# Sunefei/PathNet

Measured on AMD Instinct MI355X. Metric: paths aggregated/sec (PAGG fwd+bwd, one training step incl. on-GPU MERW sampling + Adam), higher is better.
Workload: dtype f32; 1 GPU; Cora-shaped synthetic (configs[1]): N=2708 F=1433 C=7 hid=128 path_num=40 path_len=4, 1299 masked nodes = 51960 paths/step, PathNet_homo, dropout 0.7, Adam; nodes=2708, parallelism=node-shard x1

## Files before the change

### pathnet_amd/csrc/pn_context.hip

```cpp
#include <hip/hip_runtime.h>

#include <cstdlib>
#include <cstring>
#include <map>
#include <new>
#include <vector>

#include "pn_internal.h"

struct pn_context {
    int device = 0;
    hipStream_t side = nullptr;
    hipEvent_t fork = nullptr, join = nullptr;
    int prof_mode = 0, prof_stage = -1;
    struct Rec {
        int stage;
        hipEvent_t a, b;
    };
    std::vector<Rec> recs;
    std::vector<hipEvent_t> free_events;
    std::map<const void *, int> lds_attr;
    pn::Knobs knobs;
};

namespace {

__global__ void warm_kernel() {}

__global__ void step_state_advance_kernel(pn_step_state *s) {
    if (threadIdx.x != 0 || blockIdx.x != 0) return;
    s->epoch += 1;
    s->adam_step += 1;
    uint64_t z = (s->seed += 0x9E3779B97F4A7C15ull);
    z = (z ^ (z >> 30)) * 0xBF58476D1CE4E5B9ull;
    z = (z ^ (z >> 27)) * 0x94D049BB133111EBull;
    s->seed = z ^ (z >> 31);
// ... 22 lines not shown
    (void)hipEventCreateWithFlags(&e, ctx->knobs.event_dev ? hipEventDisableSystemFence : hipEventDefault);
    return e;
}

}

namespace {

struct KnobName {
    const char *name;
    int pn::Knobs::*field;
};
const KnobName kKnobs[] = {{"PN_NODE_GEMM3", &pn::Knobs::node_gemm3}, {"PN_EVAL_ZW", &pn::Knobs::eval_zw},
                           {"PN_POOL_STEP", &pn::Knobs::pool_step}, {"PN_EVENT_DEVICE_SCOPE", &pn::Knobs::event_dev},
                           {"PN_NODE_RGRAD", &pn::Knobs::node_rgrad}, {"PN_SAMPLER_STAGE", &pn::Knobs::sampler_stage},
                           {"PN_SEQ4", &pn::Knobs::seq4}, {"PN_FC0_SPARSE", &pn::Knobs::fc0_sparse}};

}

namespace pn {

const Knobs &knobs_of(const pn_context *ctx) {
    static const Knobs defaults;
    return ctx ? ctx->knobs : defaults;
}

bool profiling_every_stage(const pn_context *ctx) { return ctx && ctx->prof_mode == 1; }

int context_check_device(const pn_context *ctx) {
    if (!ctx) return PN_OK;
    int dev = -1;
    PN_CHECK_HIP(hipGetDevice(&dev));
    if (dev != ctx->device)
        PN_FAIL(PN_ERR_ARG, "pn_context belongs to device %d, the current device is %d", ctx->device, dev);
    return PN_OK;
}

int ensure_dynamic_lds(pn_context *ctx, const void *kernel, int bytes) {
    if (ctx) {
        auto it = ctx->lds_attr.find(kernel);
        if (it != ctx->lds_attr.end() && it->second >= bytes) return PN_OK;
    }
    PN_CHECK_HIP(hipFuncSetAttribute(kernel, hipFuncAttributeMaxDynamicSharedMemorySize, bytes));
    if (ctx) ctx->lds_attr[kernel] = bytes;
    return PN_OK;
}

void *context_side_stream(pn_context *ctx) { return ctx ? (void *)ctx->side : nullptr; }
void *context_fork(pn_context *ctx, void *stream) {
    if (!ctx || !ctx->side) return nullptr;
    if (hipEventRecord(ctx->fork, (hipStream_t)stream) != hipSuccess) return nullptr;
    if (hipStreamWaitEvent(ctx->side, ctx->fork, 0) != hipSuccess) return nullptr;
    return ctx->side;
}
int context_record_join(pn_context *ctx) {
    PN_CHECK_HIP(hipEventRecord(ctx->join, ctx->side));
    return PN_OK;
}
int context_join(pn_context *ctx, void *stream) {
// ... 178 lines not shown
```

### pathnet_amd/csrc/pn_internal.h

```cpp
#pragma once
#include <cstdarg>
#include <cstdint>
#include <cstdio>

#include "../../include/pathnet_hip.h"

namespace pn {

void set_error(const char *fmt, ...) __attribute__((format(printf, 1, 2)));

#define PN_FAIL(code, ...)          \
    do {                            \
        ::pn::set_error(__VA_ARGS__); \
        return (code);              \
    } while (0)

#define PN_CHECK_HIP(expr)                                                                      \
    do {                                                                                        \
        hipError_t e_ = (expr);                                                                 \
        if (e_ != hipSuccess) PN_FAIL(PN_ERR_HIP, "%s failed: %s", #expr, hipGetErrorString(e_)); \
    } while (0)

struct GlibcPoly {
    uint32_t c[31];
// ... 4 lines not shown
GlibcPoly glibc_poly_one();
GlibcPoly glibc_poly_mul(const GlibcPoly &a, const GlibcPoly &b);
GlibcPoly glibc_poly_xpow(uint64_t d);
GlibcState glibc_apply(const GlibcPoly &p, const GlibcState &st);
GlibcState glibc_seed_state(uint32_t seed);

struct Knobs {
    int node_gemm3 = 7;
    int eval_zw = 1;
    int event_dev = 1;
    int pool_step = 1;
    int node_rgrad = 1;
    int sampler_stage = -1;
    int seq4 = 4;
    int fc0_sparse = 1;
};
const Knobs &knobs_of(const pn_context *ctx);

enum Stage {
    ST_SAMPLER_FILL = 0, ST_SAMPLER_WALK, ST_GATHER, ST_FC0, ST_BANK, ST_PLAN_PACK, ST_SEQ_FWD, ST_POOL_FWD,
    ST_FC2_GRAD, ST_POOL_BWD, ST_SEQ_BWD, ST_WGRAD, ST_BIAS_GRAD, ST_BANK_BWD, ST_FC0_BWD, ST_ZERO_FILL, ST_COUNT
};
bool profiling_every_stage(const pn_context *ctx);
int context_check_device(const pn_context *ctx);
void *context_fork(pn_context *ctx, void *stream);
void *context_side_stream(pn_context *ctx);
int context_record_join(pn_context *ctx);
int context_join(pn_context *ctx, void *stream);
int context_wait_side(pn_context *ctx, void *stream);
int ensure_dynamic_lds(pn_context *ctx, const void *kernel, int bytes);
struct StageTimer {
    StageTimer(pn_context *ctx, int stage, void *stream);
    ~StageTimer();
    pn_context *ctx;
    int slot;
    void *stream;
};

struct ZeroList {
    float *ptr[12];
    unsigned long long count[12];
    int n;
};
struct ZeroFill {
    pn_context *ctx;
// ... 24 lines not shown
```

### pathnet_amd/csrc/pn_pagg.hip

```cpp
#include <hip/hip_runtime.h>

#include <algorithm>
#include <cstdlib>
#include <cstring>
#include "pn_det.h"
#include "pn_gemm.h"
#include "pn_internal.h"
#include "pn_loss.h"
#include "pn_plan.h"
#include "pn_pool.h"
#include "pn_seq.h"
#include "pn_sparse.h"

using namespace pn;

namespace {

enum { CELL_LSTM = 1, CELL_RNN = 2, CELL_GRU = 3, CELL_MEAN = 4, CELL_SUM = 5 };
struct Dims {
    int variant, N, F, H, C, S, W, L, G, SV;
    int cell, Gw;
    int gru;
    bool generic;
    int S_total, group_begin;
// ... 80 lines not shown

inline size_t align256(size_t x) { return (x + 255) / 256 * 256; }

WsLayout ws_layout(const Dims &d) {
    WsLayout w{};
    const size_t N = d.N, H = d.H, L = d.L, G = d.G, SV = d.SV, Sb = d.Sb, Pb = (size_t)d.Sb * d.W;
    size_t at = 0;
    auto take = [&](size_t bytes) {
        size_t o = at;
        at = align256(at + bytes);
        return o;
    };
    w.Xh = take(N * H * 4);
    w.Z = take((size_t)d.ZR * H * 4);
    w.range = take(sizeof(SeqRange));
    w.wmax = take(64 * 4);
    w.Wp = take(G * H * 3 * H * 4);
    w.biasc = take(G * H * 4);
    w.WpT = take(G * H * 3 * H * 4);
    {
        const size_t rows = Pb * L, tiles = std::max<size_t>(1, ((G * H + WG_BM - 1) / WG_BM) * ((2 * H + WG_BN - 1) / WG_BN));
        const double wg_flops = 2.0 * (double)rows * (double)(G * H) * (double)(2 * H);
        size_t cus = wg_flops <= 1.2e11 ? WGRAD_CUS_SHARED : 256;
        size_t nz = (cus + tiles - 1) / tiles;
        const size_t max_nz = (rows + 4 * WG_KT - 1) / (4 * WG_KT);
        if (nz > max_nz) nz = max_nz;
        if (nz < 1) nz = 1;
        w.wgrad_split = (int)nz;
        w.wgrad_tiles = (int)tiles;
        w.wpart = take(nz * (G * H * 2 * H + G * H) * 4);
    }
// ... 282 lines not shown
    sp.L = d.L;
    sp.Pmask = d.P_total;
    sp.p_drop = a->p_seq;
    sp.seed = a->seed;
    sp.dyn = a->step_state;
    sp.mask = a->mask_seq;
    StageTimer tm(c.ctx, ST_SEQ_FWD, c.stream);
    if (!save && use_zw(c)) {
        sp.range = c.at<SeqRange>(c.w.range);
        sp.ZW = c.at<const float>(c.w.saved);
        return launch_seq_fwdzw(c.ctx, c.stream, d.H, d.Gw, sp);
    }
    if (d.math == PN_SEQ_MATH_F16X2) {
        sp.range = c.at<SeqRange>(c.w.range);
        sp.xmul = seq_xmul(a);
        return launch_seq_fwdh(c.ctx, c.stream, d.H, d.Gw, sp);
    }
    return launch_seq_fwd3(c.ctx, c.stream, d.H, d.Gw, sp);
}

PoolParams pool_fwd_params(const Call &c, int b, float *out) {
    const Dims &d = c.d;
    const pn_pagg_args *a = c.a;
    const int homo = d.variant == PN_VARIANT_HOMO;
    PoolParams pp{};
    pp.variant = d.variant;
    pp.S = c.groups(b);
    pp.W = d.W;
    pp.H = d.H;
    pp.C = d.C;
// ... 789 lines not shown
```

### pathnet_amd/csrc/pn_seq.h

```cpp
#pragma once
#include <cstdint>

#include "pn_internal.h"

namespace pn {

struct SeqRange {
    uint32_t x;
    int32_t x_esum;
    uint32_t x_cnt;
    uint32_t w_ih, w_hh;
    uint32_t dg;
};

struct SeqFwdParams {
    const float *Z;
    const int32_t *rowidx;
    const int32_t *slotof;
    const float *Wp;
    const float *biasc;
    float *hn;
    float *saved;
    float *xh;
    uint8_t *keep;
    int P, L;
    int64_t Pmask;
    float p_drop;
    uint64_t seed;
    const pn_step_state *dyn;
    const float *mask;
    const SeqRange *range;
    float xmul;
    const float *ZW;
};

struct SeqBwdParams {
    const float *saved;
    const uint8_t *keep;
    const float *dhn;
    const int32_t *rowidx, *slotof;
    const float *WpT;
    float *dG;
    float *dZ;
    int P, L;
    int merge0;
    int64_t Pmask;
    float p_drop;
    uint64_t seed;
    const float *mask;
// ... 101 lines not shown
```

### pathnet_amd/csrc/pn_seq_core.h

```cpp
#pragma once
#include <hip/hip_runtime.h>

#include <type_traits>

#include "pn_internal.h"
#include "pn_kernels.h"
#include "pn_seq.h"

namespace pn {

struct LstmFwd {
    float ig, fg, gg, og, c, h;
};
__device__ __forceinline__ LstmFwd lstm_fwd(float pi, float pf, float pg, float po, float cprev) {
    LstmFwd o;
    o.ig = sigmoidf_(pi);
    o.fg = sigmoidf_(pf);
    o.gg = tanhf_(pg);
    o.og = sigmoidf_(po);
    o.c = o.fg * cprev + o.ig * o.gg;
    o.h = o.og * tanhf_(o.c);
    return o;
}
struct GruFwd {
// ... 89 lines not shown
}
__device__ __forceinline__ float keep_dx(float dx, uint32_t keep_byte, int col, float keep_scale) {
    return (keep_byte >> (col & 3)) & 1 ? dx * keep_scale : 0.0f;
}

template <int H_, int GC_, int PLANES_>
struct SeqTile {
    static constexpr int H = H_, GC = GC_, PLANES = PLANES_;
    static constexpr int G = GC == 3 ? 4 : GC;
    static constexpr bool GRU = GC == 3;
    static constexpr int MT = 32, NW = H / 32, NT = NW * 64, GH = G * H;
    static constexpr int SV = G == 4 ? 5 : 1;
    static constexpr int FWD_PB = 4 * H + 16, FWD_PLANE = MT * FWD_PB;
    static __device__ __forceinline__ int *fwd_rowidx(unsigned char *lds) { return reinterpret_cast<int *>(lds + PLANES * FWD_PLANE); }
    static __device__ __forceinline__ int *fwd_slotof(unsigned char *lds, int L) { return fwd_rowidx(lds) + MT * L; }
    static constexpr int fwd_lds_bytes(int L) { return PLANES * FWD_PLANE + (MT * L + MT) * 4; }
    static constexpr int ZW_PB = 2 * H + 16, ZW_PLANE = MT * ZW_PB;
    static __device__ __forceinline__ int *zw_rowidx(unsigned char *lds) { return reinterpret_cast<int *>(lds + PLANES * ZW_PLANE); }
    static constexpr int zw_lds_bytes(int L) { return PLANES * ZW_PLANE + MT * L * 4; }
    static constexpr int NPASS = PLANES == 3 && G == 4 ? 2 : 1, KP = GH / NPASS;
    static constexpr int BWD_PB = 2 * KP + 16, BWD_PLANE = MT * BWD_PB, SMAX = PLANES == 2 ? 8 : 0;
    static __device__ __forceinline__ int *bwd_rowidx(unsigned char *lds) { return reinterpret_cast<int *>(lds + PLANES * BWD_PLANE); }
    static __device__ __forceinline__ int *bwd_slotof(unsigned char *lds, int L) { return bwd_rowidx(lds) + MT * L; }
    static __device__ __forceinline__ float *bwd_smax(unsigned char *lds, int L) { return reinterpret_cast<float *>(bwd_slotof(lds, L) + MT); }
    static __device__ __forceinline__ uint8_t *bwd_keep(unsigned char *lds, int L) { return reinterpret_cast<uint8_t *>(bwd_smax(lds, L) + SMAX); }
    static constexpr int bwd_lds_bytes(int L) { return PLANES * BWD_PLANE + (MT * L + MT) * 4 + SMAX * 4 + 2 * MT * (H / 4); }
};

template <class F>
int dispatch_seq(int H, int gc, F &&f) {
    auto by_h = [&](auto gcc) {
// ... 8 lines not shown
            case 256: return f(std::integral_constant<int, 256>{}, gcc);
        }
        PN_FAIL(PN_ERR_ARG, "hidden size %d not supported", H);
    };
    return gc == 3 ? by_h(std::integral_constant<int, 3>{}) : gc == 4 ? by_h(std::integral_constant<int, 4>{})
                                                                     : by_h(std::integral_constant<int, 1>{});
}

template <class... KArgs, class... Args>
int launch_with_lds(pn_context *ctx, void *stream, void (*kern)(KArgs...), dim3 grid, dim3 block, int lds_bytes, const Args &...args) {
    if (int rc = ensure_dynamic_lds(ctx, reinterpret_cast<const void *>(kern), lds_bytes)) return rc;
    hipLaunchKernelGGL(kern, grid, block, (size_t)lds_bytes, (hipStream_t)stream, args...);
    PN_CHECK_HIP(hipGetLastError());
    return PN_OK;
}
template <class T, class Params>
int launch_seq_tiles(pn_context *ctx, void *stream, void (*kern)(Params), int lds_bytes, const Params &sp) {
    return launch_with_lds(ctx, stream, kern, dim3((sp.P + T::MT - 1) / T::MT), dim3(T::NT), lds_bytes, sp);
}

}
```

### pathnet_amd/csrc/pn_seqh.hip

```cpp
#include <hip/hip_runtime.h>

#include <cstdlib>
#include <type_traits>

#include "pn_kernels.h"
#include "pn_seq.h"
#include "pn_seq_core.h"

using namespace pn;

#ifndef PN_FWDH_WAVES
#define PN_FWDH_WAVES 3
#endif
#ifndef PN_BWDH_WAVES
#define PN_BWDH_WAVES 2
#endif
#ifndef PN_TRACE_H
#define PN_TRACE_H 0
#endif
#if PN_TRACE_H
__device__ long long *g_trace_h = nullptr;
#define HSTAMP(slot)                                                                                      \
    do {                                                                                                  \
        if (g_trace_h && threadIdx.x == 0 && (slot) < 64)                                                 \
            g_trace_h[(size_t)blockIdx.x * 64 + (slot)] = (long long)__builtin_readcyclecounter();        \
    } while (0)
#define HSTAMP_RT(slot)                                                                                   \
    do {                                                                                                  \
        if (g_trace_h && threadIdx.x == 0)                                                                \
            g_trace_h[(size_t)blockIdx.x * 64 + (slot)] = (long long)__builtin_amdgcn_s_memrealtime();    \
    } while (0)
#else
#define HSTAMP(slot) do { } while (0)
#define HSTAMP_RT(slot) do { } while (0)
#endif

namespace {

typedef int i32x4 __attribute__((ext_vector_type(4)));

__device__ __forceinline__ uint32_t fbits_abs(float v) { return __float_as_uint(v) & 0x7fffffffu; }

constexpr int RANGE_PARTS = 32;
__global__ __launch_bounds__(256) void range_part_kernel(const float *__restrict__ w_ih, const float *__restrict__ w_hh, int64_t n4,
                                                         int clear_x, SeqRange *__restrict__ range, uint32_t *__restrict__ part) {
    __shared__ float red[2][4];
    const int64_t per = (n4 + RANGE_PARTS - 1) / RANGE_PARTS, lo = (int64_t)blockIdx.x * per, hi = min(n4, lo + per);
    float m0 = 0.0f, m1 = 0.0f;
    for (int64_t i = lo + threadIdx.x; i < hi; i += 256) {
        const float4 a = reinterpret_cast<const float4 *>(w_ih)[i], b = reinterpret_cast<const float4 *>(w_hh)[i];
        m0 = fmaxf(m0, fmaxf(fmaxf(fabsf(a.x), fabsf(a.y)), fmaxf(fabsf(a.z), fabsf(a.w))));
        m1 = fmaxf(m1, fmaxf(fmaxf(fabsf(b.x), fabsf(b.y)), fmaxf(fabsf(b.z), fabsf(b.w))));
    }
    m0 = wave_max(m0);
    m1 = wave_max(m1);
    if ((threadIdx.x & 63) == 0) red[0][threadIdx.x >> 6] = m0, red[1][threadIdx.x >> 6] = m1;
    __syncthreads();
    if (threadIdx.x == 0) {
        part[blockIdx.x] = __float_as_uint(fmaxf(fmaxf(red[0][0], red[0][1]), fmaxf(red[0][2], red[0][3])));
        part[RANGE_PARTS + blockIdx.x] = __float_as_uint(fmaxf(fmaxf(red[1][0], red[1][1]), fmaxf(red[1][2], red[1][3])));
        if (blockIdx.x == 0) {
            range->dg = 0u;
            if (clear_x) {
                range->x = 0u;
                range->x_esum = 0;
                range->x_cnt = 0u;
            }
        }
    }
}
__device__ __forceinline__ void range_from_parts(const uint32_t *__restrict__ part, float &m_ih, float &m_hh) {
    const int lane = threadIdx.x & 63;
    const float v = __uint_as_float(part[lane]);
    static_assert(2 * RANGE_PARTS == 64, "one partial per lane");
    float a = lane < RANGE_PARTS ? v : 0.0f, b = lane < RANGE_PARTS ? 0.0f : v;
    m_ih = wave_max(a);
    m_hh = wave_max(b);
// ... 78 lines not shown
constexpr int fwdh_waves() { return H == 32 ? 1 : H > 128 ? 2 : PN_FWDH_WAVES; }

template <int H, int GC>
__global__ __launch_bounds__(H / 32 * 64, (fwdh_waves<H>())) void seq_fwdh_kernel(SeqFwdParams p) {
    using T = SeqTile<H, GC, 2>;
    constexpr int G = T::G, MT = T::MT, NT = T::NT;
    constexpr bool GRU = T::GRU;
    constexpr bool PACKED = GC == 4;
    constexpr int SV = PACKED ? 4 : T::SV;
    constexpr int KS = H / 8, KX = KS / 2;
    constexpr int PB = T::FWD_PB, PLANE = T::FWD_PLANE;
    constexpr bool PREFETCH_X = fwdh_waves<H>() < 3, PING_PONG = PREFETCH_X;
    extern __shared__ __attribute__((aligned(16))) unsigned char ldsb[];
    int *s_rowidx = T::fwd_rowidx(ldsb);
    int *s_slotof = T::fwd_slotof(ldsb, p.L);
    const int tid = threadIdx.x, wave = tid >> 6, lane = tid & 63, li = lane & 31;
    const int q0 = __builtin_amdgcn_readfirstlane((int)blockIdx.x * MT);
    const int rows_here = __builtin_amdgcn_readfirstlane(min(MT, p.P - q0));
    const int col = 32 * wave + li;
    const int wave_u = __builtin_amdgcn_readfirstlane(wave);

    for (int i = tid; i < MT * p.L; i += NT) s_rowidx[i] = i / p.L < rows_here ? p.rowidx[(int64_t)q0 * p.L + i] : 0;
    for (int i = tid; i < MT; i += NT) s_slotof[i] = i < rows_here ? p.slotof[q0 + i] : 0;

    const FwdScales sc = fwd_scales(p.range, p.xmul);
    f32x16 cst;
#pragma unroll
    for (int r = 0; r < 16; r++) cst[r] = 0.0f;
    const float keep_scale = __int_as_float(__builtin_amdgcn_readfirstlane(__float_as_int(1.0f / (1.0f - p.p_drop))));
    const bool builtin_drop = !p.mask && p.p_drop > 0.0f;
    const uint64_t seed = p.dyn ? p.dyn->seed : p.seed;
    const size_t tile_row = (size_t)q0 * (size_t)p.L;
    uint8_t *keep_t = p.keep ? p.keep + tile_row * (H / 4) : nullptr;
    float4 *xh4_t = p.xh ? reinterpret_cast<float4 *>(p.xh) + tile_row * (2 * H / 4) : nullptr;
    float *xh_t = p.xh ? p.xh + tile_row * (2 * H) : nullptr;
    float *saved_t = p.saved ? p.saved + tile_row * (SV * H) : nullptr;
    float *hn_t = p.hn + (size_t)q0 * H;
    __syncthreads();

    constexpr int NLD = 4;
    f32x4 xr[NLD];
    uint32_t keepbits = 0;
    int tid_g = tid;
    auto gather_issue = [&](int t) {
#pragma unroll
        for (int i = 0; i < NLD; i++) {
            const int idx = tid_g + NT * i;
            const int row = idx / (H / 4), c4 = idx - row * (H / 4);
            async_load_b128(xr[i], p.Z + ((size_t)(uint32_t)s_rowidx[row * p.L + t] * (H / 4) + c4) * 4);
        }
        uint32_t bits = 0;
        if (builtin_drop) {
#pragma unroll
            for (int i = 0; i < NLD; i++) {
                const int idx = tid_g + NT * i;
                const int row = idx / (H / 4), c4 = idx - row * (H / 4);
                const float4 m = dropout4(seed, ((uint64_t)t * p.Pmask + s_slotof[row]) * (H / 4) + c4, 1u, p.p_drop);
                bits |= keep_nibble(m) << (4 * i);
            }
        }
        asm volatile("" : "+v"(bits));
        keepbits = bits;
    };
    auto gather_commit = [&](int t) {
        wait_vm<0>(xr[0], xr[1], xr[2], xr[3]);
#pragma unroll
        for (int i = 0; i < NLD; i++) {
            const int idx = tid_g + NT * i;
            const int row = idx / (H / 4), c4 = idx - row * (H / 4);
            const bool live = row < rows_here;
            float4 v = make_float4(xr[i][0], xr[i][1], xr[i][2], xr[i][3]);
            if (!live) v = make_float4(0.f, 0.f, 0.f, 0.f);
            if (p.mask) {
                if (live) {
                    const float4 m = reinterpret_cast<const float4 *>(
                        p.mask)[((int64_t)t * p.Pmask + s_slotof[row]) * (H / 4) + c4];
                    v.x *= m.x; v.y *= m.y; v.z *= m.z; v.w *= m.w;
                }
            } else if (builtin_drop) {
                const uint32_t b = keepbits >> (4 * i);
                v.x = b & 1u ? v.x * keep_scale : 0.0f;
                v.y = b & 2u ? v.y * keep_scale : 0.0f;
                v.z = b & 4u ? v.z * keep_scale : 0.0f;
                v.w = b & 8u ? v.w * keep_scale : 0.0f;
                if (keep_t && live) keep_t[((uint32_t)row * (uint32_t)p.L + t) * (uint32_t)(H / 4) + c4] = (uint8_t)(b & 15u);
            }
            uint32_t a0, a1, b0, b1;
            split2h(v.x * sc.s_x, v.y * sc.s_x, a0, a1);
            split2h(v.z * sc.s_x, v.w * sc.s_x, b0, b1);
            unsigned char *d = ldsb + row * PB + 8 * c4;
            *reinterpret_cast<uint2 *>(d) = make_uint2(a0, b0);
            *reinterpret_cast<uint2 *>(d + PLANE) = make_uint2(a1, b1);
            if (xh4_t && live) {
                float4 *xo = &at_bytes(xh4_t, (((uint32_t)row * (uint32_t)p.L + t) * (uint32_t)(2 * H / 4) + c4) * 16u);
                xo[0] = v;
                if (t == 0) xo[H / 4] = make_float4(0.f, 0.f, 0.f, 0.f);
            }
        }
    };
    gather_issue(0);
    gather_commit(0);
    __syncthreads();

    for (int t = 0; t < p.L; t++) {
        if (t == 0) HSTAMP_RT(62);
        HSTAMP(4 * t + 0);
        tid_g = wave_u * 64 + fresh_lane();
        if (PREFETCH_X && t + 1 < p.L) gather_issue(t + 1);

        f32x16 acc[G];
#pragma unroll
        for (int g = 0; g < G; g++) {
            const float bias = p.biasc[g * H + col] * sc.S;
#pragma unroll
            for (int r = 0; r < 16; r++) acc[g][r] = bias;
        }

        {
            const int nsteps = t == 0 ? KX : KS;
            const unsigned char *wb = reinterpret_cast<const unsigned char *>(p.Wp) + (size_t)wave_u * (KS * 2 * G * 1024);
            const int lane_k = fresh_lane();
            const uint32_t voff = lane_k * 16;
            const unsigned char *arow = ldsb + (lane_k & 31) * PB + 16 * (lane_k >> 5);
            u32x4 Bha[G], Bhb[G], Bl[G];
            auto load = [&](u32x4 (&B)[G], int s, int pl) {
                async_load_frags<G>(B, wb + (size_t)(s * 2 + pl) * (G * 1024), voff);
            };
            u32x4 a[2];
            auto areads = [&](int s, int pl) { a[pl] = *reinterpret_cast<const u32x4 *>(arow + 32 * s + pl * PLANE); };
            auto prod = [&](int pa, u32x4 (&B)[G]) {
#pragma unroll
                for (int g = 0; g < G; g++) acc[g] = mfma_f16(a[pa], B[g], acc[g]);
            };
            auto kstep = [&](int s, u32x4 (&Bh)[G], u32x4 (&Bhnext)[G]) {
                const int sn = min(s + 1, nsteps - 1);
                if (PING_PONG) load(Bhnext, sn, 0);
                wait_frag<(PING_PONG ? 2 : 1) * G, G>(Bh);
                prod(1, Bh);
                areads(sn, 1);
                prod(0, Bh);
                if (!PING_PONG) load(Bh, sn, 0);
                wait_frag<G, G>(Bl);
                prod(0, Bl);
                areads(sn, 0);
                load(Bl, sn, 1);
            };
            areads(0, 0);
            areads(0, 1);
            load(Bha, 0, 0);
            load(Bl, 0, 1);
#pragma unroll 1
            for (int s = 0; s < nsteps; s += 2) {
                if (PING_PONG) {
                    kstep(s, Bha, Bhb);
                    kstep(s + 1, Bhb, Bha);
                } else {
                    kstep(s, Bha, Bha);
                    kstep(s + 1, Bha, Bha);
                }
            }
            wait_frag<0, G>(Bha);
            wait_frag<0, G>(Bl);
        }
        HSTAMP(4 * t + 1);
        __syncthreads();
        HSTAMP(4 * t + 2);

        const int lane_o = fresh_lane();
        float hv[16];
#pragma unroll
        for (int r = 0; r < 16; r++) {
            const int row = acc_row(r, lane_o);
            const bool live = row < rows_here;
            float h;
            if (GRU) {
                const float hp = cst[r];
                const GruFwd c = gru_fwd(acc[0][r] * sc.inv_S, acc[G > 1 ? 1 : 0][r] * sc.inv_S, acc[G > 2 ? 2 : 0][r] * sc.inv_S,
                                         acc[G > 3 ? 3 : 0][r] * sc.inv_S, hp);
                h = c.h;
                cst[r] = h;
                if (saved_t && live) {
                    float *sv = &at_bytes(saved_t, (((uint32_t)row * (uint32_t)p.L + t) * (uint32_t)(SV * H) + col) * 4u);
                    sv[0] = c.rg; sv[H] = c.zg; sv[2 * H] = c.ng; sv[3 * H] = c.nh; sv[4 * H] = hp;
                }
            } else if (G == 4) {
                const float cprev = cst[r];
                const LstmFwd c = lstm_fwd(acc[0][r] * sc.inv_S, acc[G > 1 ? 1 : 0][r] * sc.inv_S, acc[G > 2 ? 2 : 0][r] * sc.inv_S,
                                           acc[G > 3 ? 3 : 0][r] * sc.inv_S, cprev);
                cst[r] = c.c;
                h = c.h;
                if (saved_t && live) {
                    const uint32_t base = ((uint32_t)row * (uint32_t)p.L + t) * (uint32_t)(SV * H);
                    const uint3 pk = pack_gates(c.ig, c.fg, c.gg, c.og);
                    *reinterpret_cast<uint4 *>(&at_bytes(saved_t, (base + 4u * col) * 4u)) =
                        make_uint4(pk.x, pk.y, pk.z, __float_as_uint(cprev));
                }
            } else {
                h = rnn_fwd(acc[0][r] * sc.inv_S);
                if (saved_t && live) at_bytes(saved_t, (((uint32_t)row * (uint32_t)p.L + t) * (uint32_t)H + col) * 4u) = h;
            }
            hv[r] = h;
            if (live) {
                if (t == p.L - 1)
                    at_bytes(hn_t, ((uint32_t)row * (uint32_t)H + col) * 4u) = h;
                else if (xh_t)
                    at_bytes(xh_t, (((uint32_t)row * (uint32_t)p.L + t + 1) * (uint32_t)(2 * H) + H + col) * 4u) = h;
            }
        }
        if (t + 1 < p.L) {
#pragma unroll
            for (int r = 0; r < 16; r += 2) {
                uint32_t h0, h1;
                split2h(hv[r] * sc.s_h, hv[r + 1] * sc.s_h, h0, h1);
                unsigned char *d = ldsb + acc_row(r, lane_o) * PB + 2 * (H + col);
                *reinterpret_cast<uint16_t *>(d) = (uint16_t)h0;
                *reinterpret_cast<uint16_t *>(d + PB) = (uint16_t)(h0 >> 16);
                *reinterpret_cast<uint16_t *>(d + PLANE) = (uint16_t)h1;
                *reinterpret_cast<uint16_t *>(d + PLANE + PB) = (uint16_t)(h1 >> 16);
            }
        }
        if (t + 1 < p.L) {
            tid_g = wave_u * 64 + fresh_lane();
            if (!PREFETCH_X) gather_issue(t + 1);
            gather_commit(t + 1);
            __syncthreads();
        }
        HSTAMP(4 * t + 3);
    }
    HSTAMP_RT(63);
}

template <int H, int GC>
__global__ __launch_bounds__(H / 32 * 64, (fwdh_waves<H>())) void seq_fwdzw_kernel(SeqFwdParams p) {
    using T = SeqTile<H, GC, 2>;
    constexpr int G = T::G, MT = T::MT, NT = T::NT, GH = T::GH;
    constexpr bool GRU = T::GRU;
    constexpr int KS = H / 8, KX = KS / 2, KH = KS - KX;
    constexpr int PB = T::ZW_PB, PLANE = T::ZW_PLANE;
    constexpr bool PING_PONG = fwdh_waves<H>() < 3;
    extern __shared__ __attribute__((aligned(16))) unsigned char ldsb[];
    int *s_rowidx = T::zw_rowidx(ldsb);
    const int tid = threadIdx.x, wave = tid >> 6, lane = tid & 63, li = lane & 31;
    const int q0 = blockIdx.x * MT;
    const int col = 32 * wave + li;
// ... 146 lines not shown
    constexpr bool GRU = T::GRU;
    constexpr bool PACKED = GC == 4;
    constexpr int SV = PACKED ? 4 : T::SV;
    constexpr int PB = T::BWD_PB, PLANE = T::BWD_PLANE;
    constexpr int NU = GH / 32;
    extern __shared__ __attribute__((aligned(16))) unsigned char ldsb[];
    int *s_rowidx = T::bwd_rowidx(ldsb);
    int *s_slotof = T::bwd_slotof(ldsb, p.L);
    float *s_max = T::bwd_smax(ldsb, p.L);
    uint8_t *s_keep = T::bwd_keep(ldsb, p.L);
    const int tid = threadIdx.x, wave = tid >> 6, lane = tid & 63, li = lane & 31;
    const int q0 = __builtin_amdgcn_readfirstlane((int)(gridDim.x - 1 - blockIdx.x) * MT);
    const int rows_here = __builtin_amdgcn_readfirstlane(min(MT, p.P - q0));
    const int col = 32 * wave + li;
    const int wave_u = __builtin_amdgcn_readfirstlane(wave);

    const int nidx = MT * p.L;
    auto rowidx_of = [&](int i) {
        const int rc = min(i & (MT - 1), rows_here - 1);
        return p.rowidx[((int64_t)q0 + rc) * p.L + i / MT];
    };
    const int ri0 = rowidx_of(min(tid, nidx - 1));
    const int sl0 = p.slotof[q0 + min(tid, rows_here - 1)];

    const float keep_scale = __int_as_float(__builtin_amdgcn_readfirstlane(__float_as_int(1.0f / (1.0f - p.p_drop))));
    const int e_ih = scale_exp(__uint_as_float(p.range->w_ih)), e_hh = scale_exp(__uint_as_float(p.range->w_hh));
    const size_t tile_row = (size_t)q0 * (size_t)p.L;
    const float *saved_t = p.saved + tile_row * (SV * H);
    float *dG_t = p.dG + tile_row * GH;
    const uint8_t *keep_t = p.keep ? p.keep + tile_row * (H / 4) : nullptr;
// ... 445 lines not shown
    hipLaunchKernelGGL(range_part_kernel, dim3(RANGE_PARTS), dim3(256), 0, s, w_ih, w_hh, (int64_t)Gw * H * H / 4, clear_x, range,
                       reinterpret_cast<uint32_t *>(part));
    PN_CHECK_HIP(hipGetLastError());
    const int nb = (G * H * H / 4 + 255) / 256;
    hipLaunchKernelGGL(pack_fb_kernel, dim3((unsigned)(WpT ? 2 * nb : nb)), dim3(256), 0, s, w_ih, w_hh, b_ih, b_hh, H, G, gru,
                       reinterpret_cast<const uint32_t *>(part), range, nb, reinterpret_cast<u32x4 *>(Wp), biasc,
                       reinterpret_cast<u32x4 *>(WpT));
    PN_CHECK_HIP(hipGetLastError());
    return PN_OK;
}

int launch_seq_fwdh(pn_context *ctx, void *stream, int H, int gc, const SeqFwdParams &sp) {
    if (!sp.range) PN_FAIL(PN_ERR_ARG, "seq_fwdh: operand ranges missing");
    return dispatch_seq(H, gc, [&](auto h, auto g) {
        using T = SeqTile<h.value, g.value, 2>;
        return launch_seq_tiles<T>(ctx, stream, seq_fwdh_kernel<h.value, g.value>, T::fwd_lds_bytes(sp.L), sp);
    });
}

int launch_seq_fwdzw(pn_context *ctx, void *stream, int H, int gc, const SeqFwdParams &sp) {
    if (!sp.range || !sp.ZW) PN_FAIL(PN_ERR_ARG, "seq_fwdzw: operand ranges / ZW missing");
    return dispatch_seq(H, gc, [&](auto h, auto g) {
        using T = SeqTile<h.value, g.value, 2>;
        return launch_seq_tiles<T>(ctx, stream, seq_fwdzw_kernel<h.value, g.value>, T::zw_lds_bytes(sp.L), sp);
    });
}

int launch_seq_bwdh(pn_context *ctx, void *stream, int H, int gc, const SeqBwdParams &sp) {
    if (!sp.range) PN_FAIL(PN_ERR_ARG, "seq_bwdh: operand ranges missing");
    return dispatch_seq(H, gc, [&](auto h, auto g) {
        using T = SeqTile<h.value, g.value, 2>;
// ... 12 lines not shown
```

Baseline: 61.72 million paths/s.

## Make forward sequence kernel persistent with atomic tile queue

Converts the f16x2 forward sequence kernel into a persistent kernel. The grid is sized to the resident block slots from an occupancy query, and blocks pull further tiles from a global atomic ticket counter, which resets itself when the last block leaves. The aim is to cut the tail and launch imbalance that come from launching one block per tile. In exchange it adds atomics, per-tile re-reads of kernel arguments, extra LDS for the ticket, and more register pressure from the restructured loop.

```diff
diff --git a/pathnet_amd/csrc/pn_context.hip b/pathnet_amd/csrc/pn_context.hip
--- a/pathnet_amd/csrc/pn_context.hip
+++ b/pathnet_amd/csrc/pn_context.hip
@@ -4,6 +4,7 @@
 #include <cstring>
 #include <map>
 #include <new>
+#include <utility>
 #include <vector>
 
 #include "pn_internal.h"
@@ -20,6 +21,8 @@
     std::vector<Rec> recs;
     std::vector<hipEvent_t> free_events;
     std::map<const void *, int> lds_attr;
+    std::map<std::pair<const void *, int>, int> slots;
+    int cus = 0;
     pn::Knobs knobs;
 };
 
@@ -72,7 +75,8 @@
 const KnobName kKnobs[] = {{"PN_NODE_GEMM3", &pn::Knobs::node_gemm3}, {"PN_EVAL_ZW", &pn::Knobs::eval_zw},
                            {"PN_POOL_STEP", &pn::Knobs::pool_step}, {"PN_EVENT_DEVICE_SCOPE", &pn::Knobs::event_dev},
                            {"PN_NODE_RGRAD", &pn::Knobs::node_rgrad}, {"PN_SAMPLER_STAGE", &pn::Knobs::sampler_stage},
-                           {"PN_SEQ4", &pn::Knobs::seq4}, {"PN_FC0_SPARSE", &pn::Knobs::fc0_sparse}};
+                           {"PN_SEQ4", &pn::Knobs::seq4}, {"PN_FC0_SPARSE", &pn::Knobs::fc0_sparse},
+                           {"PN_SEQ_GRID", &pn::Knobs::seq_grid}};
 
 }
 
@@ -101,6 +105,29 @@
     }
     PN_CHECK_HIP(hipFuncSetAttribute(kernel, hipFuncAttributeMaxDynamicSharedMemorySize, bytes));
     if (ctx) ctx->lds_attr[kernel] = bytes;
+    return PN_OK;
+}
+
+int resident_slots(pn_context *ctx, const void *kernel, int threads, int lds_bytes, int *slots) {
+    const std::pair<const void *, int> key(kernel, lds_bytes);
+    if (ctx) {
+        auto it = ctx->slots.find(key);
+        if (it != ctx->slots.end()) {
+            *slots = it->second;
+            return PN_OK;
+        }
+    }
+    int cus = ctx ? ctx->cus : 0;
+    if (cus <= 0) {
+        int dev = 0;
+        PN_CHECK_HIP(hipGetDevice(&dev));
+        PN_CHECK_HIP(hipDeviceGetAttribute(&cus, hipDeviceAttributeMultiprocessorCount, dev));
+        if (ctx) ctx->cus = cus;
+    }
+    int per_cu = 0;
+    PN_CHECK_HIP(hipOccupancyMaxActiveBlocksPerMultiprocessor(&per_cu, kernel, threads, (size_t)lds_bytes));
+    *slots = (per_cu > 0 ? per_cu : 1) * (cus > 0 ? cus : 1);
+    if (ctx) ctx->slots[key] = *slots;
     return PN_OK;
 }
 
diff --git a/pathnet_amd/csrc/pn_internal.h b/pathnet_amd/csrc/pn_internal.h
--- a/pathnet_amd/csrc/pn_internal.h
+++ b/pathnet_amd/csrc/pn_internal.h
@@ -42,6 +42,7 @@
     int sampler_stage = -1;
     int seq4 = 4;
     int fc0_sparse = 1;
+    int seq_grid = 0;
 };
 const Knobs &knobs_of(const pn_context *ctx);
 
@@ -57,6 +58,7 @@
 int context_join(pn_context *ctx, void *stream);
 int context_wait_side(pn_context *ctx, void *stream);
 int ensure_dynamic_lds(pn_context *ctx, const void *kernel, int bytes);
+int resident_slots(pn_context *ctx, const void *kernel, int threads, int lds_bytes, int *slots);
 struct StageTimer {
     StageTimer(pn_context *ctx, int stage, void *stream);
     ~StageTimer();
diff --git a/pathnet_amd/csrc/pn_pagg.hip b/pathnet_amd/csrc/pn_pagg.hip
--- a/pathnet_amd/csrc/pn_pagg.hip
+++ b/pathnet_amd/csrc/pn_pagg.hip
@@ -118,7 +118,7 @@
     w.Xh = take(N * H * 4);
     w.Z = take((size_t)d.ZR * H * 4);
     w.range = take(sizeof(SeqRange));
-    w.wmax = take(64 * 4);
+    w.wmax = take((64 + SEQ_QUEUE_WORDS) * 4);
     w.Wp = take(G * H * 3 * H * 4);
     w.biasc = take(G * H * 4);
     w.WpT = take(G * H * 3 * H * 4);
@@ -431,6 +431,7 @@
     if (d.math == PN_SEQ_MATH_F16X2) {
         sp.range = c.at<SeqRange>(c.w.range);
         sp.xmul = seq_xmul(a);
+        sp.queue = c.at<uint32_t>(c.w.wmax) + 64 + 2 * seq_queue_pair(b);
         return launch_seq_fwdh(c.ctx, c.stream, d.H, d.Gw, sp);
     }
     return launch_seq_fwd3(c.ctx, c.stream, d.H, d.Gw, sp);
diff --git a/pathnet_amd/csrc/pn_seq.h b/pathnet_amd/csrc/pn_seq.h
--- a/pathnet_amd/csrc/pn_seq.h
+++ b/pathnet_amd/csrc/pn_seq.h
@@ -32,7 +32,12 @@
     const SeqRange *range;
     float xmul;
     const float *ZW;
+    uint32_t *queue;
 };
+
+constexpr int SEQ_QUEUE_PAIRS = 4;
+constexpr int SEQ_QUEUE_WORDS = 2 * SEQ_QUEUE_PAIRS;
+inline int seq_queue_pair(int micro_batch) { return micro_batch & 3; }
 
 struct SeqBwdParams {
     const float *saved;
diff --git a/pathnet_amd/csrc/pn_seq_core.h b/pathnet_amd/csrc/pn_seq_core.h
--- a/pathnet_amd/csrc/pn_seq_core.h
+++ b/pathnet_amd/csrc/pn_seq_core.h
@@ -127,7 +127,8 @@
     static constexpr int FWD_PB = 4 * H + 16, FWD_PLANE = MT * FWD_PB;
     static __device__ __forceinline__ int *fwd_rowidx(unsigned char *lds) { return reinterpret_cast<int *>(lds + PLANES * FWD_PLANE); }
     static __device__ __forceinline__ int *fwd_slotof(unsigned char *lds, int L) { return fwd_rowidx(lds) + MT * L; }
-    static constexpr int fwd_lds_bytes(int L) { return PLANES * FWD_PLANE + (MT * L + MT) * 4; }
+    static __device__ __forceinline__ uint32_t *fwd_ticket(unsigned char *lds, int L) { return reinterpret_cast<uint32_t *>(fwd_slotof(lds, L) + MT); }
+    static constexpr int fwd_lds_bytes(int L) { return PLANES * FWD_PLANE + (MT * L + MT) * 4 + 4; }
     static constexpr int ZW_PB = 2 * H + 16, ZW_PLANE = MT * ZW_PB;
     static __device__ __forceinline__ int *zw_rowidx(unsigned char *lds) { return reinterpret_cast<int *>(lds + PLANES * ZW_PLANE); }
     static constexpr int zw_lds_bytes(int L) { return PLANES * ZW_PLANE + MT * L * 4; }
@@ -166,9 +167,24 @@
     PN_CHECK_HIP(hipGetLastError());
     return PN_OK;
 }
-template <class T, class Params>
+template <class T, bool PERSISTENT = false, class Params>
 int launch_seq_tiles(pn_context *ctx, void *stream, void (*kern)(Params), int lds_bytes, const Params &sp) {
-    return launch_with_lds(ctx, stream, kern, dim3((sp.P + T::MT - 1) / T::MT), dim3(T::NT), lds_bytes, sp);
+    const int ntiles = (sp.P + T::MT - 1) / T::MT;
+    if constexpr (!PERSISTENT) {
+        return launch_with_lds(ctx, stream, kern, dim3(ntiles), dim3(T::NT), lds_bytes, sp);
+    } else {
+    if (int rc = ensure_dynamic_lds(ctx, reinterpret_cast<const void *>(kern), lds_bytes)) return rc;
+    const int knob = knobs_of(ctx).seq_grid;
+    int grid = ntiles;
+    if (knob > 0) {
+        grid = knob;
+    } else if (knob == 0 && sp.queue) {
+        if (int rc = resident_slots(ctx, reinterpret_cast<const void *>(kern), T::NT, lds_bytes, &grid)) return rc;
+    }
+    Params q = sp;
+    if (grid >= ntiles || !sp.queue) grid = ntiles, q.queue = nullptr;
+    return launch_with_lds(ctx, stream, kern, dim3(grid), dim3(T::NT), lds_bytes, q);
+    }
 }
 
 }
diff --git a/pathnet_amd/csrc/pn_seqh.hip b/pathnet_amd/csrc/pn_seqh.hip
--- a/pathnet_amd/csrc/pn_seqh.hip
+++ b/pathnet_amd/csrc/pn_seqh.hip
@@ -20,17 +20,19 @@
 #endif
 #if PN_TRACE_H
 __device__ long long *g_trace_h = nullptr;
+#define HSTAMP_ROW(ticket) const size_t trace_row = (ticket)
 #define HSTAMP(slot)                                                                                      \
     do {                                                                                                  \
         if (g_trace_h && threadIdx.x == 0 && (slot) < 64)                                                 \
-            g_trace_h[(size_t)blockIdx.x * 64 + (slot)] = (long long)__builtin_readcyclecounter();        \
+            g_trace_h[trace_row * 64 + (slot)] = (long long)__builtin_readcyclecounter();                 \
     } while (0)
 #define HSTAMP_RT(slot)                                                                                   \
     do {                                                                                                  \
         if (g_trace_h && threadIdx.x == 0)                                                                \
-            g_trace_h[(size_t)blockIdx.x * 64 + (slot)] = (long long)__builtin_amdgcn_s_memrealtime();    \
+            g_trace_h[trace_row * 64 + (slot)] = (long long)__builtin_amdgcn_s_memrealtime();             \
     } while (0)
 #else
+#define HSTAMP_ROW(ticket) do { } while (0)
 #define HSTAMP(slot) do { } while (0)
 #define HSTAMP_RT(slot) do { } while (0)
 #endif
@@ -40,6 +42,19 @@
 typedef int i32x4 __attribute__((ext_vector_type(4)));
 
 __device__ __forceinline__ uint32_t fbits_abs(float v) { return __float_as_uint(v) & 0x7fffffffu; }
+
+template <class P>
+__device__ __forceinline__ const P __attribute__((address_space(4))) *kernarg_fresh() {
+    auto kp = (const P __attribute__((address_space(4))) *)__builtin_amdgcn_kernarg_segment_ptr();
+    asm volatile("" : "+s"(kp));
+    return kp;
+}
+__device__ __forceinline__ void queue_leave(uint32_t *q) {
+    if (!q || threadIdx.x != 0) return;
+    if (__hip_atomic_fetch_add(q + 1, 1u, __ATOMIC_RELAXED, __HIP_MEMORY_SCOPE_AGENT) + 1u != gridDim.x) return;
+    __hip_atomic_store(q, 0u, __ATOMIC_RELAXED, __HIP_MEMORY_SCOPE_AGENT);
+    __hip_atomic_store(q + 1, 0u, __ATOMIC_RELAXED, __HIP_MEMORY_SCOPE_AGENT);
+}
 
 constexpr int RANGE_PARTS = 32;
 __global__ __launch_bounds__(256) void range_part_kernel(const float *__restrict__ w_ih, const float *__restrict__ w_hh, int64_t n4,
@@ -61,6 +76,7 @@
         part[RANGE_PARTS + blockIdx.x] = __float_as_uint(fmaxf(fmaxf(red[1][0], red[1][1]), fmaxf(red[1][2], red[1][3])));
         if (blockIdx.x == 0) {
             range->dg = 0u;
+            for (int i = 0; i < SEQ_QUEUE_WORDS; i++) part[2 * RANGE_PARTS + i] = 0u;
             if (clear_x) {
                 range->x = 0u;
                 range->x_esum = 0;
@@ -169,220 +185,241 @@
     extern __shared__ __attribute__((aligned(16))) unsigned char ldsb[];
     int *s_rowidx = T::fwd_rowidx(ldsb);
     int *s_slotof = T::fwd_slotof(ldsb, p.L);
-    const int tid = threadIdx.x, wave = tid >> 6, lane = tid & 63, li = lane & 31;
-    const int q0 = __builtin_amdgcn_readfirstlane((int)blockIdx.x * MT);
-    const int rows_here = __builtin_amdgcn_readfirstlane(min(MT, p.P - q0));
-    const int col = 32 * wave + li;
-    const int wave_u = __builtin_amdgcn_readfirstlane(wave);
-
-    for (int i = tid; i < MT * p.L; i += NT) s_rowidx[i] = i / p.L < rows_here ? p.rowidx[(int64_t)q0 * p.L + i] : 0;
-    for (int i = tid; i < MT; i += NT) s_slotof[i] = i < rows_here ? p.slotof[q0 + i] : 0;
-
+    uint32_t *s_ticket = T::fwd_ticket(ldsb, p.L);
+    const int wave_u = __builtin_amdgcn_readfirstlane((int)threadIdx.x >> 6);
     const FwdScales sc = fwd_scales(p.range, p.xmul);
-    f32x16 cst;
-#pragma unroll
-    for (int r = 0; r < 16; r++) cst[r] = 0.0f;
     const float keep_scale = __int_as_float(__builtin_amdgcn_readfirstlane(__float_as_int(1.0f / (1.0f - p.p_drop))));
-    const bool builtin_drop = !p.mask && p.p_drop > 0.0f;
-    const uint64_t seed = p.dyn ? p.dyn->seed : p.seed;
-    const size_t tile_row = (size_t)q0 * (size_t)p.L;
-    uint8_t *keep_t = p.keep ? p.keep + tile_row * (H / 4) : nullptr;
-    float4 *xh4_t = p.xh ? reinterpret_cast<float4 *>(p.xh) + tile_row * (2 * H / 4) : nullptr;
-    float *xh_t = p.xh ? p.xh + tile_row * (2 * H) : nullptr;
-    float *saved_t = p.saved ? p.saved + tile_row * (SV * H) : nullptr;
-    float *hn_t = p.hn + (size_t)q0 * H;
-    __syncthreads();
-
-    constexpr int NLD = 4;
-    f32x4 xr[NLD];
-    uint32_t keepbits = 0;
-    int tid_g = tid;
-    auto gather_issue = [&](int t) {
-#pragma unroll
-        for (int i = 0; i < NLD; i++) {
-            const int idx = tid_g + NT * i;
-            const int row = idx / (H / 4), c4 = idx - row * (H / 4);
-            async_load_b128(xr[i], p.Z + ((size_t)(uint32_t)s_rowidx[row * p.L + t] * (H / 4) + c4) * 4);
-        }
-        uint32_t bits = 0;
-        if (builtin_drop) {
-#pragma unroll
+    const uint32_t ntiles = (uint32_t)(p.P + MT - 1) / MT;
+    const bool persistent = p.queue != nullptr;
+    uint32_t tile = blockIdx.x;
+#pragma unroll 1
+    for (;;) {
+        const int lane = fresh_lane(), tid = wave_u * 64 + lane, col = 32 * wave_u + (lane & 31);
+        const auto *kp = kernarg_fresh<SeqFwdParams>();
+        const int q0 = __builtin_amdgcn_readfirstlane((int)tile * MT);
+        const int rows_here = __builtin_amdgcn_readfirstlane(min(MT, kp->P - q0));
+        HSTAMP_ROW(tile);
+
+        for (int i = tid; i < MT * p.L; i += NT) s_rowidx[i] = i / p.L < rows_here ? kp->rowidx[(int64_t)q0 * p.L + i] : 0;
+        for (int i = tid; i < MT; i += NT) s_slotof[i] = i < rows_here ? kp->slotof[q0 + i] : 0;
+
+        f32x16 cst;
+    #pragma unroll
+        for (int r = 0; r < 16; r++) cst[r] = 0.0f;
+        const size_t tile_row = (size_t)q0 * (size_t)p.L;
+        uint8_t *keep_t = kp->keep ? kp->keep + tile_row * (H / 4) : nullptr;
+        float4 *xh4_t = kp->xh ? reinterpret_cast<float4 *>(kp->xh) + tile_row * (2 * H / 4) : nullptr;
+        float *xh_t = kp->xh ? kp->xh + tile_row * (2 * H) : nullptr;
+        float *saved_t = kp->saved ? kp->saved + tile_row * (SV * H) : nullptr;
+        float *hn_t = kp->hn + (size_t)q0 * H;
+        uint32_t next_tile = ntiles;
+        __syncthreads();
+
+        constexpr int NLD = 4;
+        f32x4 xr[NLD];
+        uint32_t keepbits = 0;
+        int tid_g = tid;
+        auto gather_issue = [&](int t) {
+            const auto *kg = kernarg_fresh<SeqFwdParams>();
+    #pragma unroll
             for (int i = 0; i < NLD; i++) {
                 const int idx = tid_g + NT * i;
                 const int row = idx / (H / 4), c4 = idx - row * (H / 4);
-                const float4 m = dropout4(seed, ((uint64_t)t * p.Pmask + s_slotof[row]) * (H / 4) + c4, 1u, p.p_drop);
-                bits |= keep_nibble(m) << (4 * i);
-            }
-        }
-        asm volatile("" : "+v"(bits));
-        keepbits = bits;
-    };
-    auto gather_commit = [&](int t) {
-        wait_vm<0>(xr[0], xr[1], xr[2], xr[3]);
-#pragma unroll
-        for (int i = 0; i < NLD; i++) {
-            const int idx = tid_g + NT * i;
-            const int row = idx / (H / 4), c4 = idx - row * (H / 4);
-            const bool live = row < rows_here;
-            float4 v = make_float4(xr[i][0], xr[i][1], xr[i][2], xr[i][3]);
-            if (!live) v = make_float4(0.f, 0.f, 0.f, 0.f);
-            if (p.mask) {
+                async_load_b128(xr[i], kg->Z + ((size_t)(uint32_t)s_rowidx[row * p.L + t] * (H / 4) + c4) * 4);
+            }
+            uint32_t bits = 0;
+            if (!kg->mask && kg->p_drop > 0.0f) {
+                const uint64_t seed = kg->dyn ? kg->dyn->seed : kg->seed;
+    #pragma unroll
+                for (int i = 0; i < NLD; i++) {
+                    const int idx = tid_g + NT * i;
+                    const int row = idx / (H / 4), c4 = idx - row * (H / 4);
+                    const float4 m = dropout4(seed, ((uint64_t)t * kg->Pmask + s_slotof[row]) * (H / 4) + c4, 1u, kg->p_drop);
+                    bits |= keep_nibble(m) << (4 * i);
+                }
+            }
+            asm volatile("" : "+v"(bits));
+            keepbits = bits;
+        };
+        auto gather_commit = [&](int t) {
+            const auto *kc = kernarg_fresh<SeqFwdParams>();
+            const float *mask = kc->mask;
+            wait_vm<0>(xr[0], xr[1], xr[2], xr[3]);
+    #pragma unroll
+            for (int i = 0; i < NLD; i++) {
+                const int idx = tid_g + NT * i;
+                const int row = idx / (H / 4), c4 = idx - row * (H / 4);
+                const bool live = row < rows_here;
+                float4 v = make_float4(xr[i][0], xr[i][1], xr[i][2], xr[i][3]);
+                if (!live) v = make_float4(0.f, 0.f, 0.f, 0.f);
+                if (mask) {
+                    if (live) {
+                        const float4 m = reinterpret_cast<const float4 *>(
+                            mask)[((int64_t)t * kc->Pmask + s_slotof[row]) * (H / 4) + c4];
+                        v.x *= m.x; v.y *= m.y; v.z *= m.z; v.w *= m.w;
+                    }
+                } else if (kc->p_drop > 0.0f) {
+                    const uint32_t b = keepbits >> (4 * i);
+                    v.x = b & 1u ? v.x * keep_scale : 0.0f;
+                    v.y = b & 2u ? v.y * keep_scale : 0.0f;
+                    v.z = b & 4u ? v.z * keep_scale : 0.0f;
+                    v.w = b & 8u ? v.w * keep_scale : 0.0f;
+                    if (keep_t && live) keep_t[((uint32_t)row * (uint32_t)p.L + t) * (uint32_t)(H / 4) + c4] = (uint8_t)(b & 15u);
+                }
+                uint32_t a0, a1, b0, b1;
+                split2h(v.x * sc.s_x, v.y * sc.s_x, a0, a1);
+                split2h(v.z * sc.s_x, v.w * sc.s_x, b0, b1);
+                unsigned char *d = ldsb + row * PB + 8 * c4;
+                *reinterpret_cast<uint2 *>(d) = make_uint2(a0, b0);
+                *reinterpret_cast<uint2 *>(d + PLANE) = make_uint2(a1, b1);
+                if (xh4_t && live) {
+                    float4 *xo = &at_bytes(xh4_t, (((uint32_t)row * (uint32_t)p.L + t) * (uint32_t)(2 * H / 4) + c4) * 16u);
+                    xo[0] = v;
+                    if (t == 0) xo[H / 4] = make_float4(0.f, 0.f, 0.f, 0.f);
+                }
+            }
+        };
+        gather_issue(0);
+        gather_commit(0);
+        __syncthreads();
+
+        for (int t = 0; t < p.L; t++) {
+            if (t == 0) HSTAMP_RT(62);
+            HSTAMP(4 * t + 0);
+            tid_g = wave_u * 64 + fresh_lane();
+            if (PREFETCH_X && t + 1 < p.L) gather_issue(t + 1);
+            const bool draw = persistent && t == p.L - 1;
+            uint32_t ticket = 0;
+            if (draw && tid == 0)
+                ticket = gridDim.x + __hip_atomic_fetch_add(kernarg_fresh<SeqFwdParams>()->queue, 1u, __ATOMIC_RELAXED, __HIP_MEMORY_SCOPE_AGENT);
+
+            const auto *kk = kernarg_fresh<SeqFwdParams>();
+            f32x16 acc[G];
+    #pragma unroll
+            for (int g = 0; g < G; g++) {
+                const float bias = kk->biasc[g * H + col] * sc.S;
+    #pragma unroll
+                for (int r = 0; r < 16; r++) acc[g][r] = bias;
+            }
+
+            {
+                const int nsteps = t == 0 ? KX : KS;
+                const unsigned char *wb = reinterpret_cast<const unsigned char *>(kk->Wp) + (size_t)wave_u * (KS * 2 * G * 1024);
+                const int lane_k = fresh_lane();
+                const uint32_t voff = lane_k * 16;
+                const unsigned char *arow = ldsb + (lane_k & 31) * PB + 16 * (lane_k >> 5);
+                u32x4 Bha[G], Bhb[G], Bl[G];
+                auto load = [&](u32x4 (&B)[G], int s, int pl) {
+                    async_load_frags<G>(B, wb + (size_t)(s * 2 + pl) * (G * 1024), voff);
+                };
+                u32x4 a[2];
+                auto areads = [&](int s, int pl) { a[pl] = *reinterpret_cast<const u32x4 *>(arow + 32 * s + pl * PLANE); };
+                auto prod = [&](int pa, u32x4 (&B)[G]) {
+    #pragma unroll
+                    for (int g = 0; g < G; g++) acc[g] = mfma_f16(a[pa], B[g], acc[g]);
+                };
+                auto kstep = [&](int s, u32x4 (&Bh)[G], u32x4 (&Bhnext)[G]) {
+                    const int sn = min(s + 1, nsteps - 1);
+                    if (PING_PONG) load(Bhnext, sn, 0);
+                    wait_frag<(PING_PONG ? 2 : 1) * G, G>(Bh);
+                    prod(1, Bh);
+                    areads(sn, 1);
+                    prod(0, Bh);
+                    if (!PING_PONG) load(Bh, sn, 0);
+                    wait_frag<G, G>(Bl);
+                    prod(0, Bl);
+                    areads(sn, 0);
+                    load(Bl, sn, 1);
+                };
+                areads(0, 0);
+                areads(0, 1);
+                load(Bha, 0, 0);
+                load(Bl, 0, 1);
+    #pragma unroll 1
+                for (int s = 0; s < nsteps; s += 2) {
+                    if (PING_PONG) {
+                        kstep(s, Bha, Bhb);
+                        kstep(s + 1, Bhb, Bha);
+                    } else {
+                        kstep(s, Bha, Bha);
+                        kstep(s + 1, Bha, Bha);
+                    }
+                }
+                wait_frag<0, G>(Bha);
+                wait_frag<0, G>(Bl);
+            }
+            HSTAMP(4 * t + 1);
+            if (draw && tid == 0) *s_ticket = ticket;
+            __syncthreads();
+            HSTAMP(4 * t + 2);
+            if (draw) next_tile = __builtin_amdgcn_readfirstlane(*s_ticket);
+
+            const int lane_o = fresh_lane();
+            float hv[16];
+    #pragma unroll
+            for (int r = 0; r < 16; r++) {
+                const int row = acc_row(r, lane_o);
+                const bool live = row < rows_here;
+                float h;
+                if (GRU) {
+                    const float hp = cst[r];
+                    const GruFwd c = gru_fwd(acc[0][r] * sc.inv_S, acc[G > 1 ? 1 : 0][r] * sc.inv_S, acc[G > 2 ? 2 : 0][r] * sc.inv_S,
+                                             acc[G > 3 ? 3 : 0][r] * sc.inv_S, hp);
+                    h = c.h;
+                    cst[r] = h;
+                    if (saved_t && live) {
+                        float *sv = &at_bytes(saved_t, (((uint32_t)row * (uint32_t)p.L + t) * (uint32_t)(SV * H) + col) * 4u);
+                        sv[0] = c.rg; sv[H] = c.zg; sv[2 * H] = c.ng; sv[3 * H] = c.nh; sv[4 * H] = hp;
+                    }
+                } else if (G == 4) {
+                    const float cprev = cst[r];
+                    const LstmFwd c = lstm_fwd(acc[0][r] * sc.inv_S, acc[G > 1 ? 1 : 0][r] * sc.inv_S, acc[G > 2 ? 2 : 0][r] * sc.inv_S,
+                                               acc[G > 3 ? 3 : 0][r] * sc.inv_S, cprev);
+                    cst[r] = c.c;
+                    h = c.h;
+                    if (saved_t && live) {
+                        const uint32_t base = ((uint32_t)row * (uint32_t)p.L + t) * (uint32_t)(SV * H);
+                        const uint3 pk = pack_gates(c.ig, c.fg, c.gg, c.og);
+                        *reinterpret_cast<uint4 *>(&at_bytes(saved_t, (base + 4u * col) * 4u)) =
+                            make_uint4(pk.x, pk.y, pk.z, __float_as_uint(cprev));
+                    }
+                } else {
+                    h = rnn_fwd(acc[0][r] * sc.inv_S);
+                    if (saved_t && live) at_bytes(saved_t, (((uint32_t)row * (uint32_t)p.L + t) * (uint32_t)H + col) * 4u) = h;
+                }
+                hv[r] = h;
                 if (live) {
-                    const float4 m = reinterpret_cast<const float4 *>(
-                        p.mask)[((int64_t)t * p.Pmask + s_slotof[row]) * (H / 4) + c4];
-                    v.x *= m.x; v.y *= m.y; v.z *= m.z; v.w *= m.w;
-                }
-            } else if (builtin_drop) {
-                const uint32_t b = keepbits >> (4 * i);
-                v.x = b & 1u ? v.x * keep_scale : 0.0f;
-                v.y = b & 2u ? v.y * keep_scale : 0.0f;
-                v.z = b & 4u ? v.z * keep_scale : 0.0f;
-                v.w = b & 8u ? v.w * keep_scale : 0.0f;
-                if (keep_t && live) keep_t[((uint32_t)row * (uint32_t)p.L + t) * (uint32_t)(H / 4) + c4] = (uint8_t)(b & 15u);
-            }
-            uint32_t a0, a1, b0, b1;
-            split2h(v.x * sc.s_x, v.y * sc.s_x, a0, a1);
-            split2h(v.z * sc.s_x, v.w * sc.s_x, b0, b1);
-            unsigned char *d = ldsb + row * PB + 8 * c4;
-            *reinterpret_cast<uint2 *>(d) = make_uint2(a0, b0);
-            *reinterpret_cast<uint2 *>(d + PLANE) = make_uint2(a1, b1);
-            if (xh4_t && live) {
-                float4 *xo = &at_bytes(xh4_t, (((uint32_t)row * (uint32_t)p.L + t) * (uint32_t)(2 * H / 4) + c4) * 16u);
-                xo[0] = v;
-                if (t == 0) xo[H / 4] = make_float4(0.f, 0.f, 0.f, 0.f);
-            }
-        }
-    };
-    gather_issue(0);
-    gather_commit(0);
-    __syncthreads();
-
-    for (int t = 0; t < p.L; t++) {
-        if (t == 0) HSTAMP_RT(62);
-        HSTAMP(4 * t + 0);
-        tid_g = wave_u * 64 + fresh_lane();
-        if (PREFETCH_X && t + 1 < p.L) gather_issue(t + 1);
-
-        f32x16 acc[G];
-#pragma unroll
-        for (int g = 0; g < G; g++) {
-            const float bias = p.biasc[g * H + col] * sc.S;
-#pragma unroll
-            for (int r = 0; r < 16; r++) acc[g][r] = bias;
-        }
-
-        {
-            const int nsteps = t == 0 ? KX : KS;
-            const unsigned char *wb = reinterpret_cast<const unsigned char *>(p.Wp) + (size_t)wave_u * (KS * 2 * G * 1024);
-            const int lane_k = fresh_lane();
-            const uint32_t voff = lane_k * 16;
-            const unsigned char *arow = ldsb + (lane_k & 31) * PB + 16 * (lane_k >> 5);
-            u32x4 Bha[G], Bhb[G], Bl[G];
-            auto load = [&](u32x4 (&B)[G], int s, int pl) {
-                async_load_frags<G>(B, wb + (size_t)(s * 2 + pl) * (G * 1024), voff);
-            };
-            u32x4 a[2];
-            auto areads = [&](int s, int pl) { a[pl] = *reinterpret_cast<const u32x4 *>(arow + 32 * s + pl * PLANE); };
-            auto prod = [&](int pa, u32x4 (&B)[G]) {
-#pragma unroll
-                for (int g = 0; g < G; g++) acc[g] = mfma_f16(a[pa], B[g], acc[g]);
-            };
-            auto kstep = [&](int s, u32x4 (&Bh)[G], u32x4 (&Bhnext)[G]) {
-                const int sn = min(s + 1, nsteps - 1);
-                if (PING_PONG) load(Bhnext, sn, 0);
-                wait_frag<(PING_PONG ? 2 : 1) * G, G>(Bh);
-                prod(1, Bh);
-                areads(sn, 1);
-                prod(0, Bh);
-                if (!PING_PONG) load(Bh, sn, 0);
-                wait_frag<G, G>(Bl);
-                prod(0, Bl);
-                areads(sn, 0);
-                load(Bl, sn, 1);
-            };
-            areads(0, 0);
-            areads(0, 1);
-            load(Bha, 0, 0);
-            load(Bl, 0, 1);
-#pragma unroll 1
-            for (int s = 0; s < nsteps; s += 2) {
-                if (PING_PONG) {
-                    kstep(s, Bha, Bhb);
-                    kstep(s + 1, Bhb, Bha);
-                } else {
-                    kstep(s, Bha, Bha);
-                    kstep(s + 1, Bha, Bha);
-                }
-            }
-            wait_frag<0, G>(Bha);
-            wait_frag<0, G>(Bl);
-        }
-        HSTAMP(4 * t + 1);
-        __syncthreads();
-        HSTAMP(4 * t + 2);
-
-        const int lane_o = fresh_lane();
-        float hv[16];
-#pragma unroll
-        for (int r = 0; r < 16; r++) {
-            const int row = acc_row(r, lane_o);
-            const bool live = row < rows_here;
-            float h;
-            if (GRU) {
-                const float hp = cst[r];
-                const GruFwd c = gru_fwd(acc[0][r] * sc.inv_S, acc[G > 1 ? 1 : 0][r] * sc.inv_S, acc[G > 2 ? 2 : 0][r] * sc.inv_S,
-                                         acc[G > 3 ? 3 : 0][r] * sc.inv_S, hp);
-                h = c.h;
-                cst[r] = h;
-                if (saved_t && live) {
-                    float *sv = &at_bytes(saved_t, (((uint32_t)row * (uint32_t)p.L + t) * (uint32_t)(SV * H) + col) * 4u);
-                    sv[0] = c.rg; sv[H] = c.zg; sv[2 * H] = c.ng; sv[3 * H] = c.nh; sv[4 * H] = hp;
-                }
-            } else if (G == 4) {
-                const float cprev = cst[r];
-                const LstmFwd c = lstm_fwd(acc[0][r] * sc.inv_S, acc[G > 1 ? 1 : 0][r] * sc.inv_S, acc[G > 2 ? 2 : 0][r] * sc.inv_S,
-                                           acc[G > 3 ? 3 : 0][r] * sc.inv_S, cprev);
-                cst[r] = c.c;
-                h = c.h;
-                if (saved_t && live) {
-                    const uint32_t base = ((uint32_t)row * (uint32_t)p.L + t) * (uint32_t)(SV * H);
-                    const uint3 pk = pack_gates(c.ig, c.fg, c.gg, c.og);
-                    *reinterpret_cast<uint4 *>(&at_bytes(saved_t, (base + 4u * col) * 4u)) =
-                        make_uint4(pk.x, pk.y, pk.z, __float_as_uint(cprev));
-                }
-            } else {
-                h = rnn_fwd(acc[0][r] * sc.inv_S);
-                if (saved_t && live) at_bytes(saved_t, (((uint32_t)row * (uint32_t)p.L + t) * (uint32_t)H + col) * 4u) = h;
-            }
-            hv[r] = h;
-            if (live) {
-                if (t == p.L - 1)
-                    at_bytes(hn_t, ((uint32_t)row * (uint32_t)H + col) * 4u) = h;
-                else if (xh_t)
-                    at_bytes(xh_t, (((uint32_t)row * (uint32_t)p.L + t + 1) * (uint32_t)(2 * H) + H + col) * 4u) = h;
-            }
-        }
-        if (t + 1 < p.L) {
-#pragma unroll
-            for (int r = 0; r < 16; r += 2) {
-                uint32_t h0, h1;
-                split2h(hv[r] * sc.s_h, hv[r + 1] * sc.s_h, h0, h1);
-                unsigned char *d = ldsb + acc_row(r, lane_o) * PB + 2 * (H + col);
-                *reinterpret_cast<uint16_t *>(d) = (uint16_t)h0;
-                *reinterpret_cast<uint16_t *>(d + PB) = (uint16_t)(h0 >> 16);
-                *reinterpret_cast<uint16_t *>(d + PLANE) = (uint16_t)h1;
-                *reinterpret_cast<uint16_t *>(d + PLANE + PB) = (uint16_t)(h1 >> 16);
-            }
-        }
-        if (t + 1 < p.L) {
-            tid_g = wave_u * 64 + fresh_lane();
-            if (!PREFETCH_X) gather_issue(t + 1);
-            gather_commit(t + 1);
-            __syncthreads();
-        }
-        HSTAMP(4 * t + 3);
-    }
-    HSTAMP_RT(63);
+                    if (t == p.L - 1)
+                        at_bytes(hn_t, ((uint32_t)row * (uint32_t)H + col) * 4u) = h;
+                    else if (xh_t)
+                        at_bytes(xh_t, (((uint32_t)row * (uint32_t)p.L + t + 1) * (uint32_t)(2 * H) + H + col) * 4u) = h;
+                }
+            }
+            if (t + 1 < p.L) {
+    #pragma unroll
+                for (int r = 0; r < 16; r += 2) {
+                    uint32_t h0, h1;
+                    split2h(hv[r] * sc.s_h, hv[r + 1] * sc.s_h, h0, h1);
+                    unsigned char *d = ldsb + acc_row(r, lane_o) * PB + 2 * (H + col);
+                    *reinterpret_cast<uint16_t *>(d) = (uint16_t)h0;
+                    *reinterpret_cast<uint16_t *>(d + PB) = (uint16_t)(h0 >> 16);
+                    *reinterpret_cast<uint16_t *>(d + PLANE) = (uint16_t)h1;
+                    *reinterpret_cast<uint16_t *>(d + PLANE + PB) = (uint16_t)(h1 >> 16);
+                }
+            }
+            if (t + 1 < p.L) {
+                tid_g = wave_u * 64 + fresh_lane();
+                if (!PREFETCH_X) gather_issue(t + 1);
+                gather_commit(t + 1);
+                __syncthreads();
+            }
+            HSTAMP(4 * t + 3);
+        }
+        HSTAMP_RT(63);
+        tile = next_tile;
+        if (tile >= ntiles) break;
+    }
+    queue_leave(kernarg_fresh<SeqFwdParams>()->queue);
 }
 
 template <int H, int GC>
@@ -559,6 +596,7 @@
     const int rows_here = __builtin_amdgcn_readfirstlane(min(MT, p.P - q0));
     const int col = 32 * wave + li;
     const int wave_u = __builtin_amdgcn_readfirstlane(wave);
+    HSTAMP_ROW(blockIdx.x);
 
     const int nidx = MT * p.L;
     auto rowidx_of = [&](int i) {
@@ -1034,7 +1072,7 @@
     if (!sp.range) PN_FAIL(PN_ERR_ARG, "seq_fwdh: operand ranges missing");
     return dispatch_seq(H, gc, [&](auto h, auto g) {
         using T = SeqTile<h.value, g.value, 2>;
-        return launch_seq_tiles<T>(ctx, stream, seq_fwdh_kernel<h.value, g.value>, T::fwd_lds_bytes(sp.L), sp);
+        return launch_seq_tiles<T, true>(ctx, stream, seq_fwdh_kernel<h.value, g.value>, T::fwd_lds_bytes(sp.L), sp);
     });
 }
 
```

After: 59.45 million paths/s. 0.963x the previous value.
